# marcelm/cutadapt

Hardware: NVIDIA H100
Metric: reads/sec (150bp SE, 1 adapter, e=0.1) (higher is better)
Workload: dtype u8

## Files before the change

cutadapt_b200/csrc/cg_api.cu:

```cuda
#include <cuda_runtime.h>
#include <stdio.h>
#include <stdlib.h>
#include <string.h>

#include <algorithm>
#include <chrono>
#include <map>
#include <memory>
#include <string>
#include <type_traits>
#include <vector>

#include "../../include/cutadapt_b200.h"
#include "cg_hostpack.h"
#include <array>

#include "cg_gzip_core.cuh"
#include "cg_kernels.cuh"
#include "cg_jit.h"
#include "cg_setbuild.h"

static_assert(sizeof(cg_match) == 32 && sizeof(cg_match_rec) == 32, "cg_match must be 32 bytes");
static_assert(sizeof(CgAdapter) == 80 && sizeof(CgEntry) == 32 && sizeof(CgGroup) == 32 &&
                  sizeof(CgSetHeader) == 80, "table layout");

static thread_local std::string g_err;

static int fail(int code, const std::string &msg)
{
    g_err = msg;
    return code;
}
static int cuda_fail(cudaError_t e, const char *what)
{
    char buf[256];
    snprintf(buf, sizeof buf, "CUDA error in %s: %s", what, cudaGetErrorString(e));
    g_err = buf;
    return e == cudaErrorMemoryAllocation ? CG_ENOMEM : CG_ECUDA;
}
#define CU(x)                                                  \
    do {                                                       \
        cudaError_t _e = (x);                                  \
        if (_e != cudaSuccess) return cuda_fail(_e, #x);       \
    } while (0)

extern "C" int cg_version(void) { return CG_ABI_VERSION; }
extern "C" const char *cg_last_error(void) { return g_err.c_str(); }

template <class T, bool Pinned> class GrowBuf {
  public:
    T *p = nullptr;
    size_t cap = 0;
    GrowBuf() = default;
    GrowBuf(const GrowBuf &) = delete;
    GrowBuf &operator=(const GrowBuf &) = delete;
    GrowBuf(GrowBuf &&o) noexcept : p(o.p), cap(o.cap) { o.p = nullptr; o.cap = 0; }
    GrowBuf &operator=(GrowBuf &&o) noexcept
    {
        if (this != &o) {
            release();
            p = o.p; cap = o.cap;
            o.p = nullptr; o.cap = 0;
        }
        return *this;
    }
    ~GrowBuf() { release(); }
    int ensure(size_t n)
    {
        if (n <= cap) return CG_OK;
        release();
        size_t want = n + n / 4 + 64;
        cudaError_t e = Pinned ? cudaMallocHost((void **)&p, want * sizeof(T)) : cudaMalloc((void **)&p, want * sizeof(T));
        if (e != cudaSuccess) return cuda_fail(e, Pinned ? "cudaMallocHost" : "cudaMalloc");
        cap = want;
        return CG_OK;
    }

  private:
    void release()
    {
        if (p) Pinned ? cudaFreeHost(p) : cudaFree(p);
        p = nullptr; cap = 0;
    }
};
template <class T> using DevBuf = GrowBuf<T, false>;
template <class T> using PinBuf = GrowBuf<T, true>;
static_assert(!std::is_copy_constructible<DevBuf<uint8_t>>::value && !std::is_copy_constructible<PinBuf<uint8_t>>::value,
              "buffers own their memory: move them");

#define CG_N_LANES 3
struct Lane {
    cudaStream_t stream = nullptr;
    DevBuf<uint8_t> d_seq, d_qual, d_pack;
    DevBuf<uint64_t> d_exc;
    PinBuf<uint8_t> h_pack;
    PinBuf<uint64_t> h_exc;
    DevBuf<int64_t> d_offs;
    DevBuf<cg_match_rec> d_out;
    DevBuf<int32_t> d_qtrim;
    PinBuf<uint8_t> h_seq, h_qual;
    PinBuf<int64_t> h_offs;
    PinBuf<cg_match_rec> h_out;
    PinBuf<int32_t> h_qtrim;
    bool busy = false;
    cg_match_rec *dst_out = nullptr; size_t n_out = 0; bool out_bounced = false;
    int32_t *dst_qtrim = nullptr; size_t n_qtrim = 0; bool qtrim_bounced = false;
};

#define CG_ROWS_KINDS 3
struct FqRows {
    bool requested = false;
    bool gzip = false;
    int32_t n_entries = 0;
    std::vector<char> text;
    std::vector<int32_t> text_off;
    int64_t limit = -1;
    DevBuf<uint8_t> d_text, d_out, d_gz;
    DevBuf<int32_t> d_textoff, d_row;
    DevBuf<int64_t> d_rowoff;
    int64_t bytes = 0, bytes_plain = 0;
};

#define CG_FQ_SLOTS 4
struct FastqSlot {
    cudaStream_t stream = nullptr;
    bool busy = false;
    int64_t n_bytes = 0;
    DevBuf<uint8_t> d_in, d_out, d_seq, d_qual;
    DevBuf<uint32_t> d_tiles, d_nl;
    DevBuf<CgFastqRecord> d_rec;
    DevBuf<int32_t> d_len, d_interval, d_keep, d_outlen, d_qtrim, d_mask, d_adest, d_dmbytes, d_dest, d_pairkey, d_origin;
    DevBuf<uint8_t> d_destkeep;
    FqRows rows[CG_ROWS_KINDS];
    bool rows_ready = false;
    DevBuf<int64_t> d_dmbase;
    DevBuf<int64_t> d_offs, d_outoff;
    DevBuf<unsigned long long> d_scan;
    DevBuf<cg_match_rec> d_matches, d_matches_rc;
    DevBuf<uint8_t> d_isrc;
    DevBuf<uint8_t> d_norm;
    DevBuf<int32_t> d_faline;
    DevBuf<int64_t> d_faoff;
    DevBuf<unsigned long long> d_fqstats;
    DevBuf<int32_t> d_polya;
    PinBuf<unsigned long long> h_fqstats;
    DevBuf<int32_t> d_fold;
    DevBuf<unsigned long long> d_ilverr;
    DevBuf<CgGzPiece> d_gzpieces;
    DevBuf<uint8_t> d_gzslots, d_gzout;
    DevBuf<int32_t> d_gzsizes;
    DevBuf<int64_t> d_gzoff;
    int ilv = 0, ilv_peer = -1, ilv_format = 0;
    DevBuf<unsigned long long> d_counters;
    DevBuf<int> d_err;
    PinBuf<uint8_t> h_in, h_out;
    PinBuf<unsigned long long> h_counters;
};

struct GzinStream {
    DevBuf<uint8_t> d_gz, d_plain;
    PinBuf<uint8_t> h_gz;
    DevBuf<int32_t> d_counts, d_cand, d_members, d_flag;
    DevBuf<int64_t> d_offs;
    DevBuf<GuMember> d_res;
    DevBuf<long long> d_moff;
    DevBuf<unsigned long long> d_scan, d_small;
    DevBuf<uint32_t> d_tiles, d_nl;
    cudaEvent_t done = nullptr;
    long long carry = 0, consumed = 0, members = 0;
    long long pend_plain = 0, pend_consumed = 0, pend_members = 0;
    bool split = false;
    long long stride = CG_GZIN_STRIDE;
    struct Member { int in = 0, bitoff = 0, trailer = 0; uint32_t crc = 0; long long len = 0, start = 0; } mem, pmem;
    long long pend_respec = 0;
    DevBuf<uint8_t> d_win, d_pwin, d_wins;
    DevBuf<GuChunk> d_ch;
    DevBuf<long long> d_coff, d_room;
    DevBuf<uint16_t> d_sym;
    DevBuf<int32_t> d_redo;
    DevBuf<uint32_t> d_part;
    ~GzinStream() { if (done) cudaEventDestroy(done); }
};

struct FqStatsAcc {
    int32_t n_adapters = 0, max_len = 0, kmax = 0;
    std::vector<int64_t> v;
};

struct cg_ctx {
    int device = 0;
    cudaStream_t stream = nullptr;
    bool own_stream = false;
    int sm_count = 148;
    size_t smem_optin = 0;
    Lane lanes[CG_N_LANES];
    int *d_err = nullptr;
    uint8_t *d_enc = nullptr;
    double *d_phred = nullptr;
    DevBuf<uint32_t> scratch_p;
    DevBuf<int> scratch_w;
    DevBuf<unsigned long long> d_stats;
    DevBuf<uint4> tasks;
    DevBuf<uint4> tasks2, tasks3;
    DevBuf<uint2> stat_ents;
    unsigned long long *d_task_count = nullptr;
    DevBuf<cg_match_rec> pass_tmp;
    DevBuf<int32_t> view_base, view_back;
    long long launches = 0;
    std::vector<std::pair<cudaEvent_t, cudaEvent_t>> timing;
    std::vector<cudaEvent_t> event_pool;
    double timed_ms = 0.0;
    long long timed_n = 0;
    std::vector<std::array<cudaEvent_t, 4>> stage_events;
    double stage_ms[3] = {0, 0, 0};
    CgHostPool *pool = nullptr;
    std::vector<std::vector<uint64_t>> exc_scratch;
    long long h2d_bytes = 0, d2h_bytes = 0;
    double prof[8] = {0, 0, 0, 0, 0, 0, 0, 0};
    double pack_fraction = 0.6;
    double pack_ref_fraction = 0.6, pack_ref_rate = 0.0;
    int pack_dir = +1;
    bool pack_have_ref = false;
    int numa_node = -1;
    cudaEvent_t scratch_ev = nullptr;
    cudaStream_t scratch_stream = nullptr;
    bool scratch_busy = false;
    FastqSlot fq[CG_FQ_SLOTS];
    int fq_next = 0;
    std::map<int32_t, FqStatsAcc> fq_stats;
    int32_t fq_stats_next = 1;
    std::map<int32_t, GzinStream> gzin;
    int32_t gzin_next = 1;
};

struct cg_adapterset {
    cg_ctx *ctx = nullptr;
    CgBuiltSet host;
    uint8_t *d_blob = nullptr;
    uint64_t *d_masks = nullptr;
    CgEntry *d_entries = nullptr;
    uint8_t *d_index = nullptr;
    struct Pass {
        cg_adapterset *sub = nullptr;
        int group = 0, role = 0;
        int front_pass = -1;
        int map_off = 0;
    };
    std::vector<Pass> passes;
    std::vector<int32_t> pass_map;
    int32_t *d_pass_map = nullptr;
    CgSelectTables select_tables;
    mutable CgJitKernel *jit[2][2][2] = {};
    mutable int jit_state[2][2][2] = {};
    mutable long long plane_reads = 0;
    mutable std::string jit_error;
};

extern "C" int cg_ctx_create(int device, void *stream, cg_ctx **out)
{
    if (!out) return fail(CG_EINVAL, "cg_ctx_create: out is NULL");
    int count = 0;
    cudaError_t e = cudaGetDeviceCount(&count);
    if (e != cudaSuccess || count == 0)
        return fail(CG_ECUDA, std::string("no usable CUDA device (") + cudaGetErrorString(e) +
                                  "); cutadapt_b200 has no CPU fallback");
    if (device < 0 || device >= count) return fail(CG_EINVAL, "cg_ctx_create: device ordinal out of range");
    CU(cudaSetDevice(device));
    std::unique_ptr<cg_ctx, decltype(&cg_ctx_destroy)> c(new cg_ctx(), cg_ctx_destroy);
    c->device = device;
    cudaDeviceProp prop;
    CU(cudaGetDeviceProperties(&prop, device));
    c->sm_count = prop.multiProcessorCount;
    c->smem_optin = prop.sharedMemPerBlockOptin;
    if (stream) { c->stream = (cudaStream_t)stream; c->own_stream = false; }
    else { CU(cudaStreamCreateWithFlags(&c->stream, cudaStreamNonBlocking)); c->own_stream = true; }
    for (int i = 0; i < CG_N_LANES; ++i) CU(cudaStreamCreateWithFlags(&c->lanes[i].stream, cudaStreamNonBlocking));
    CU(cudaEventCreateWithFlags(&c->scratch_ev, cudaEventDisableTiming));
    CU(cudaMalloc((void **)&c->d_err, 16 * sizeof(int)));
    CU(cudaMemset(c->d_err, 0, 16 * sizeof(int)));
    CU(cudaMalloc((void **)&c->d_task_count, 64));
    CU(cudaMemset(c->d_task_count, 0, 64));
    CU(cudaMalloc((void **)&c->d_enc, 768));
    uint8_t enc[768];
    cg_build_enc_tables(enc);
    CU(cudaMemcpy(c->d_enc, enc, 768, cudaMemcpyHostToDevice));
    {
        double phred[256];
        cg_build_phred_table(phred);
        CU(cudaMalloc((void **)&c->d_phred, sizeof phred));
        CU(cudaMemcpy(c->d_phred, phred, sizeof phred, cudaMemcpyHostToDevice));
    }
    *out = c.release();
    return CG_OK;
}

static void resolve_timing(cg_ctx *c)
{
    for (auto &pr : c->timing) {
        float ms = 0.f;
        if (cudaEventSynchronize(pr.second) == cudaSuccess && cudaEventElapsedTime(&ms, pr.first, pr.second) == cudaSuccess) {
            c->timed_ms += ms; c->timed_n += 1;
        }
        c->event_pool.push_back(pr.first);
        c->event_pool.push_back(pr.second);
    }
    c->timing.clear();
}

extern "C" int cg_ctx_destroy(cg_ctx *c)
{
    if (!c) return CG_OK;
    cudaSetDevice(c->device);
    cudaDeviceSynchronize();
    resolve_timing(c);
    for (auto ev : c->event_pool) cudaEventDestroy(ev);
    delete c->pool;
    c->pool = nullptr;
    for (Lane &l : c->lanes)
        if (l.stream) cudaStreamDestroy(l.stream);
    for (FastqSlot &f : c->fq)
        if (f.stream) cudaStreamDestroy(f.stream);
    if (c->scratch_ev) cudaEventDestroy(c->scratch_ev);
    if (c->d_task_count) cudaFree(c->d_task_count);
    if (c->d_err) cudaFree(c->d_err);
    if (c->d_enc) cudaFree(c->d_enc);
    if (c->d_phred) cudaFree(c->d_phred);
    if (c->own_stream && c->stream) cudaStreamDestroy(c->stream);
    delete c;
    return CG_OK;
}

extern "C" int cg_ctx_synchronize(cg_ctx *c)
{
    if (!c) return fail(CG_EINVAL, "ctx is NULL");
    CU(cudaSetDevice(c->device));
    CU(cudaStreamSynchronize(c->stream));
    for (int i = 0; i < CG_N_LANES; ++i) CU(cudaStreamSynchronize(c->lanes[i].stream));
    return CG_OK;
}

extern "C" int64_t cg_ctx_launch_count(cg_ctx *c) { return c ? c->launches : 0; }

extern "C" int cg_ctx_stage_times(cg_ctx *c, double *out3, int reset)
{
    if (!c || !out3) return fail(CG_EINVAL, "cg_ctx_stage_times: NULL argument");
    CU(cudaSetDevice(c->device));
    for (auto &e : c->stage_events) {
        CU(cudaEventSynchronize(e[3]));
        for (int i = 0; i < 3; ++i) {
            float ms = 0;
            CU(cudaEventElapsedTime(&ms, e[i], e[i + 1]));
            c->stage_ms[i] += ms;
        }
        for (auto ev : e) cudaEventDestroy(ev);
    }
    c->stage_events.clear();
    for (int i = 0; i < 3; ++i) out3[i] = c->stage_ms[i];
    if (reset) c->stage_ms[0] = c->stage_ms[1] = c->stage_ms[2] = 0;
    return CG_OK;
}

extern "C" int cg_ctx_kernel_time(cg_ctx *c, double *total_ms, int64_t *launches, int reset)
{
    if (!c) return fail(CG_EINVAL, "ctx is NULL");
    CU(cudaSetDevice(c->device));
    resolve_timing(c);
    if (total_ms) *total_ms = c->timed_ms;
    if (launches) *launches = c->timed_n;
    if (reset) { c->timed_ms = 0.0; c->timed_n = 0; }
    return CG_OK;
}

static void destroy_passes(cg_adapterset *s)
{
    for (auto &p : s->passes) cg_adapterset_destroy(p.sub);
    s->passes.clear();
    s->pass_map.clear();
    if (s->d_pass_map) { cudaFree(s->d_pass_map); s->d_pass_map = nullptr; }
}

static int upload_set(cg_ctx *c, cg_adapterset *s)
{
    s->ctx = c;
    cudaError_t e = cudaSetDevice(c->device);
    if (e == cudaSuccess) e = cudaMalloc((void **)&s->d_blob, s->host.blob.size());
    if (e == cudaSuccess) e = cudaMemcpy(s->d_blob, s->host.blob.data(), s->host.blob.size(), cudaMemcpyHostToDevice);
    if (e == cudaSuccess) e = cudaMalloc((void **)&s->d_masks, s->host.masks64.size() * 8);
    if (e == cudaSuccess) e = cudaMemcpy(s->d_masks, s->host.masks64.data(), s->host.masks64.size() * 8, cudaMemcpyHostToDevice);
    if (e == cudaSuccess && !s->host.index_blob.empty()) {
        e = cudaMalloc((void **)&s->d_index, s->host.index_blob.size());
        if (e == cudaSuccess) e = cudaMemcpy(s->d_index, s->host.index_blob.data(), s->host.index_blob.size(), cudaMemcpyHostToDevice);
    }
    if (e != cudaSuccess) {
        if (s->d_blob) cudaFree(s->d_blob);
        if (s->d_masks) cudaFree(s->d_masks);
        if (s->d_index) cudaFree(s->d_index);
        s->d_blob = nullptr; s->d_masks = nullptr; s->d_index = nullptr;
        return cuda_fail(e, "adapter set upload");
    }
    return CG_OK;
}

extern "C" int cg_adapterset_create_indexed(cg_ctx *c, const cg_adapter_desc *adapters, int32_t n_adapters,
                                            const cg_group_desc *groups, int32_t n_groups,
                                            const cg_index_desc *indexes, int32_t n_indexes, cg_adapterset **out)
{
    if (!c || !out) return fail(CG_EINVAL, "cg_adapterset_create: NULL argument");
    cg_adapterset *s = new cg_adapterset();
    std::string err;
    int rc = cg_build_set(adapters, n_adapters, groups, n_groups, s->host, err, indexes, n_indexes);
    if (rc != CG_OK) { delete s; return fail(rc, err); }
    rc = upload_set(c, s);
    if (rc != CG_OK) { delete s; return rc; }
    CgMultiPlan plan;
    if (cg_plan_passes(adapters, n_adapters, groups, n_groups, indexes, n_indexes, plan, err) == CG_OK &&
        !plan.passes.empty()) {
        bool ok = true;
        for (auto &pp : plan.passes) {
            cg_adapterset::Pass P;
            P.group = pp.group; P.role = pp.role; P.front_pass = pp.front_pass; P.map_off = pp.map_off;
            P.sub = new cg_adapterset();
            P.sub->host = std::move(pp.set);
            if (upload_set(c, P.sub) != CG_OK) { delete P.sub; ok = false; break; }
            s->passes.push_back(P);
        }
        if (ok) {
            const CgSetHeader *H = (const CgSetHeader *)s->host.blob.data();
            cg_fill_select_tables((const CgGroup *)(s->host.blob.data() + H->groups_off), s->host.n_groups,
                                  s->host.slots, plan.passes, s->select_tables);
            s->pass_map = plan.pass_map;
            cudaError_t e = cudaMalloc((void **)&s->d_pass_map, s->pass_map.size() * sizeof(int32_t));
            if (e == cudaSuccess)
                e = cudaMemcpy(s->d_pass_map, s->pass_map.data(), s->pass_map.size() * sizeof(int32_t), cudaMemcpyHostToDevice);
            if (e != cudaSuccess) { cudaGetLastError(); ok = false; }
        }
        if (!ok) destroy_passes(s);
    }
    *out = s;
    return CG_OK;
}

extern "C" int cg_adapterset_create(cg_ctx *c, const cg_adapter_desc *adapters, int32_t n_adapters,
                                    const cg_group_desc *groups, int32_t n_groups, cg_adapterset **out)
{
    return cg_adapterset_create_indexed(c, adapters, n_adapters, groups, n_groups, nullptr, 0, out);
}

extern "C" int cg_adapterset_destroy(cg_adapterset *s)
{
    if (!s) return CG_OK;
    if (s->ctx) cudaSetDevice(s->ctx->device);
    if (s->d_blob) cudaFree(s->d_blob);
    if (s->d_masks) cudaFree(s->d_masks);
    if (s->d_index) cudaFree(s->d_index);
    for (int w = 0; w < 2; ++w)
        for (int q = 0; q < 2; ++q)
            for (int v = 0; v < 2; ++v) cg_jit_destroy(s->jit[w][q][v]);
    destroy_passes(s);
    delete s;
    return CG_OK;
}

extern "C" int cg_adapterset_jit_status(const cg_adapterset *s)
{
    if (!s) return 0;
    const cg_adapterset *t = (!s->passes.empty() && s->passes[0].sub) ? s->passes[0].sub : s;
    int st = 0;
    for (int w = 0; w < 2; ++w)
        for (int q = 0; q < 2; ++q)
            for (int v = 0; v < 2; ++v) {
                if (t->jit_state[w][q][v] == 1) st = 1;
                else if (t->jit_state[w][q][v] == -1 && st == 0) st = -1;
            }
    if (st == -1) g_err = "first-stage specialisation failed: " + t->jit_error;
    return st;
}

extern "C" int64_t cg_adapterset_jit_source(const cg_adapterset *s, int32_t plane_words, int32_t has_qual, int32_t stats,
                                            char *buf, int64_t cap)
{
    if (!s) return 0;
    const std::string src = cg_jit_pscan_source(s->host, plane_words, has_qual != 0, stats != 0);
    if (buf && cap > 0) {
        const size_t n = std::min<size_t>(src.size(), (size_t)cap - 1);
        memcpy(buf, src.data(), n);
        buf[n] = 0;
    }
    return (int64_t)src.size();
}

extern "C" int cg_adapterset_slots(const cg_adapterset *s) { return s ? s->host.slots : 0; }

extern "C" int cg_adapterset_effective_length(const cg_adapterset *s, int32_t adapter, int32_t *out)
{
    if (!s || !out || adapter < 0 || adapter >= s->host.n_adapters) return fail(CG_EINVAL, "bad adapter index");
    *out = s->host.effective_length[adapter];
    return CG_OK;
}

struct TrimSwitches {
    static bool is(const char *name, const char *value) { const char *e = getenv(name); return e && strcmp(e, value) == 0; }
    static long long at_least_1024(const char *e) { const long long v = e ? atoll(e) : 0; return v >= 1024 ? v : 0; }
    bool force_general = is("CUTADAPT_B200_KERNEL", "general");
    bool force_block = is("CUTADAPT_B200_KERNEL", "block");
    bool force_warp = is("CUTADAPT_B200_KERNEL", "warp");
    bool shiftand = is("CUTADAPT_B200_SCAN", "shiftand");
    bool no_band = getenv("CUTADAPT_B200_NO_BAND") != nullptr;
    bool no_light = getenv("CUTADAPT_B200_NO_LIGHT") != nullptr;
    bool no_index_kernel = getenv("CUTADAPT_B200_NO_INDEX_KERNEL") != nullptr;
    bool two_lists = getenv("CUTADAPT_B200_TWO_LISTS") != nullptr;
    bool task_bytes = getenv("CUTADAPT_B200_TASK_BYTES") != nullptr;
    bool no_band_lists = getenv("CUTADAPT_B200_NO_BAND_LISTS") != nullptr;
    bool stage_times = getenv("CUTADAPT_B200_STAGE_TIMES") != nullptr;
    bool jit_never = is("CUTADAPT_B200_JIT", "0"), jit_always = is("CUTADAPT_B200_JIT", "1");
    long long sub_reads = at_least_1024(getenv("CUTADAPT_B200_SUB_READS"));
};

struct StatsRequest { unsigned long long *d_stats; int max_len, kmax; };

enum class TrimKind { Index, Light, Split, Warp, Fast, Generic, MultiPass };

struct TrimSchedule {
    TrimKind kind = TrimKind::Generic;
    int tile_cap = 0, mini_cap = 0, carry_slot = 0;
    size_t smem = 0;
    int occ = 0;
    bool simple = false;
    size_t list_smem = 0;
    int plan_occ = 0, run_occ = 0;
    int plane_w = 0, plane_rec = 0;
    long long sub = 0;
    CgJitKernel *jit = nullptr;
    int jit_occ = 0;
    bool fuse_stats = false;
};

static int choose_schedule(cg_ctx *c, const cg_adapterset *s, int64_t n_reads, int max_read_len, const cg_params *p,
                           bool has_view, const StatsRequest *stats, const TrimSwitches &sw, TrimSchedule &d)
{
    const CgBuiltSet &h = s->host;
    const int times = p->times < 1 ? 1 : p->times;
    const bool want_q = p->quality_trim != 0 || p->nextseq_trim != 0;
    if (!s->passes.empty() && times == 1 && !sw.force_general) {
        d.kind = TrimKind::MultiPass;
        d.sub = sw.sub_reads ? sw.sub_reads : 32LL << 20;
        return CG_OK;
    }
    if (h.all_indexed && !want_q && !h.any_wide && h.max_m + 1 <= CG_LIGHT_ROWS && !sw.force_general && !sw.no_light) {
        d.kind = times == 1 && !has_view && h.slots == 1 && !sw.no_index_kernel ? TrimKind::Index : TrimKind::Light;
        d.sub = 64LL << 20;
        return CG_OK;
    }
    const uint32_t blob_bytes = (uint32_t)h.blob.size();
    const long long tile_cap = ((long long)CG_NT * max_read_len + 32 + 15) / 16 * 16;
    bool fast = !h.any_wide && max_read_len <= CG_PACKED_MAX_N && tile_cap < (1 << 24);
    if (fast) {
        d.tile_cap = (int)tile_cap;
        d.smem = cg_fast_smem_bytes(blob_bytes, d.tile_cap, h.max_m + 1, want_q);
        fast = d.smem <= c->smem_optin;
    }
    d.simple = fast && h.simple_ok && times == 1 && !sw.force_general;
    if (fast) {
        CU(cg_fast_occupancy(want_q, d.simple, d.smem, &d.occ));
        fast = d.occ >= 1;
    }
    d.kind = fast ? TrimKind::Fast : TrimKind::Generic;
    const long long mini = ((long long)32 * max_read_len + 32 + 15) / 16 * 16;
    if (d.simple && h.max_m <= 32 && sw.force_warp && mini < (1 << 20)) {
        d.mini_cap = (int)mini;
        d.carry_slot = (int)(((long long)max_read_len + 4 + 15) / 16 * 16 + 16);
        const size_t wsmem = cg_warp_smem_bytes(blob_bytes, d.mini_cap, d.carry_slot, want_q);
        int wocc = 0;
        if (wsmem <= c->smem_optin) CU(cg_warp_occupancy(want_q, wsmem, &wocc));
        if (wocc >= 1) { d.kind = TrimKind::Warp; d.smem = wsmem; d.occ = wocc; }
        return CG_OK;
    }
    if (!d.simple || h.max_m > 64 || sw.force_block || sw.force_warp || mini >= (1 << 20)) return CG_OK;
    const CgSetHeader *hdr = (const CgSetHeader *)h.blob.data();
    if (hdr->plane_count > 0 && max_read_len <= 256 && !sw.shiftand) d.plane_w = max_read_len <= 160 ? 5 : 8;
    const long long cslot = ((long long)max_read_len + 4 + 15) / 16 * 16 + 32;
    d.mini_cap = (int)mini;
    d.carry_slot = (int)(d.plane_w ? std::max<long long>(cslot, 16LL * (2 * d.plane_w + 1) + 16) : cslot);
    size_t scan_smem = d.plane_w ? cg_pscan_smem_bytes(blob_bytes, d.mini_cap, want_q)
                                 : cg_scan_smem_bytes(blob_bytes, d.mini_cap, want_q);
    d.list_smem = cg_dp_smem_bytes(blob_bytes, d.carry_slot);
    if (scan_smem > c->smem_optin || d.list_smem > c->smem_optin) return CG_OK;
    int scan_occ = 0;
    if (d.plane_w) CU(cg_pscan_occupancy(want_q, d.plane_w, false, scan_smem, &scan_occ));
    else CU(cg_scan_occupancy(want_q, scan_smem, &scan_occ));
    CU(cg_list_occupancy(true, h.max_m, false, d.list_smem, &d.plan_occ));
    CU(cg_list_occupancy(false, h.max_m, false, d.list_smem, &d.run_occ));
    if (scan_occ < 1 || d.plan_occ < 1 || d.run_occ < 1) return CG_OK;
    if (d.plane_w && stats && !has_view && h.n_adapters == 1 && times == 1 && h.slots == 1 && !want_q && !sw.two_lists &&
        stats->max_len <= 4096 && cg_stats_entries_smem_bytes(stats->max_len, stats->kmax) <= 48 * 1024) {
        const size_t fsmem = cg_pscan_smem_bytes(blob_bytes, d.mini_cap, want_q, stats->max_len);
        int focc = 0;
        if (fsmem <= c->smem_optin) CU(cg_pscan_occupancy(want_q, d.plane_w, true, fsmem, &focc));
        int pocc = 0, rocc = 0;
        CU(cg_list_occupancy(true, h.max_m, true, d.list_smem, &pocc));
        CU(cg_list_occupancy(false, h.max_m, true, d.list_smem, &rocc));
        d.fuse_stats = focc >= 1 && focc >= scan_occ && pocc >= d.plan_occ && rocc >= d.run_occ;
        if (d.fuse_stats) { scan_smem = fsmem; scan_occ = focc; }
    }
    if (d.plane_w) {
        const int wi = d.plane_w <= 5 ? 0 : 1, qi = want_q ? 1 : 0, vi = d.fuse_stats ? 1 : 0;
        s->plane_reads += n_reads;
        if (!sw.jit_never && s->jit_state[wi][qi][vi] == 0 && (sw.jit_always || s->plane_reads >= (4LL << 20))) {
            std::string err;
            s->jit[wi][qi][vi] = cg_jit_build_pscan(h, d.plane_w, want_q, d.fuse_stats, err);
            s->jit_state[wi][qi][vi] = s->jit[wi][qi][vi] ? 1 : -1;
            if (!s->jit[wi][qi][vi]) s->jit_error = err;
        }
        if (!sw.jit_never && s->jit_state[wi][qi][vi] == 1) {
            d.jit_occ = cg_jit_occupancy(s->jit[wi][qi][vi], CG_NT, scan_smem);
            if (d.jit_occ >= 1) d.jit = s->jit[wi][qi][vi];
        }
    }
    d.kind = TrimKind::Split;
    d.smem = scan_smem; d.occ = scan_occ;
    d.sub = sw.sub_reads ? sw.sub_reads : (d.plane_w && sw.task_bytes) ? (16LL << 20) : (32LL << 20);
    d.sub = std::min<long long>(d.sub, 1LL << 31);
    d.plane_rec = d.plane_w ? (sw.task_bytes ? 4 + 2 * d.plane_w + 1 : 4) : 2;
    return CG_OK;
}

static int trim_grid(const cg_ctx *c, int blocks_per_sm, long long need)
{
    return (int)std::max<long long>(1, std::min<long long>((long long)blocks_per_sm * c->sm_count, need));
}

static int launch_index(cg_ctx *c, const CgKernelArgs &a, const TrimSchedule &d, cudaStream_t st)
{
    int rc = c->tasks.ensure((size_t)((std::min<long long>(a.n_reads, d.sub) + 3) / 4));
    if (rc != CG_OK) return rc;
    for (long long r0 = 0; r0 < a.n_reads; r0 += d.sub) {
        const long long n_sub = std::min<long long>(d.sub, a.n_reads - r0);
        CgKernelArgs b = a;
        b.offsets = a.offsets + r0; b.n_reads = n_sub; b.out = a.out + (size_t)r0 * a.slots;
        b.tasks = c->tasks.p; b.task_count = c->d_task_count;
        CU(cudaMemsetAsync(c->d_task_count, 0, sizeof(unsigned long long), st));
        CU(cg_launch_index(b, trim_grid(c, 16, (n_sub + CG_NT - 1) / CG_NT), st));
        c->launches += 2;
    }
    return CG_OK;
}

static int launch_split(cg_ctx *c, const cg_adapterset *s, const CgKernelArgs &a, const TrimSchedule &d,
                        const TrimSwitches &sw, cudaStream_t st)
{
    const long long cap = std::min<long long>(a.n_reads, d.sub);
    int rc = c->tasks.ensure((size_t)cap * d.plane_rec);
    if (rc == CG_OK) rc = c->tasks2.ensure((size_t)cap * 4);
    if (rc == CG_OK) rc = c->tasks3.ensure((size_t)cap * 4);
    if (rc == CG_OK && d.fuse_stats) rc = c->stat_ents.ensure((size_t)cap);
    if (rc != CG_OK) return rc;
    unsigned long long *cnt = c->d_task_count;
    for (long long r0 = 0; r0 < a.n_reads; r0 += d.sub) {
        const long long n_sub = std::min<long long>(d.sub, a.n_reads - r0);
        CgKernelArgs b = a;
        b.offsets = a.offsets + r0;
        b.n_reads = n_sub;
        b.out = a.out + (size_t)r0 * a.times * a.slots;
        b.qtrim = a.qtrim ? a.qtrim + 2 * r0 : nullptr;
        b.view = a.view ? a.view + 2 * r0 : nullptr;
        b.task_cap = n_sub;
        CU(cudaMemsetAsync(cnt, 0, 8 * sizeof(unsigned long long), st));
        const long long need = ((n_sub + 31) / 32 + 3) / 4;
        std::array<cudaEvent_t, 4> sev = {nullptr, nullptr, nullptr, nullptr};
        if (sw.stage_times && c->stage_events.size() < 4096) {
            for (auto &e : sev) CU(cudaEventCreate(&e));
            CU(cudaEventRecord(sev[0], st));
        }
        b.tasks = c->tasks.p; b.task_count = cnt;
        b.task_rec = d.plane_rec;
        b.task_count_b = (d.plane_w && sw.two_lists) ? cnt + 4 : nullptr;
        if (d.plane_w && d.jit) {
            const int rcj = cg_jit_launch(d.jit, trim_grid(c, d.jit_occ, need), CG_NT, d.smem, (void *)st, &b);
            if (rcj != 0) return fail(CG_ECUDA, "launch of the specialised first stage failed (CUresult " + std::to_string(rcj) + ")");
        }
        else if (d.plane_w) CU(cg_launch_pscan(b, a.quality_trim != 0, d.plane_w, trim_grid(c, d.occ, need), d.smem, st));
        else CU(cg_launch_scan(b, a.quality_trim != 0, trim_grid(c, d.occ, need), d.smem, st));
        if (sev[0]) CU(cudaEventRecord(sev[1], st));
        b.stat_ents = c->stat_ents.p; b.stat_count = cnt + 6;
        b.tasks2 = c->tasks2.p; b.task2_count = cnt + 1;
        b.tasks3 = c->tasks3.p; b.task3_count = cnt + 2;
        b.task2_count_b = (CG_RUN_BAND && d.plane_w && !sw.no_band_lists) ? cnt + 5 : nullptr;
        CU(cg_launch_list(b, true, s->host.max_m, trim_grid(c, d.plan_occ, need), d.list_smem, st));
        c->launches += 2;
        if (d.plane_w) {
            CgKernelArgs b2 = b;
            b2.tasks = c->tasks3.p; b2.task_count = cnt + 2; b2.task_rec = 2;
            b2.tasks3 = nullptr; b2.task3_count = cnt + 3; b2.task_count_b = nullptr;
            CU(cg_launch_list(b2, true, s->host.max_m, trim_grid(c, d.plan_occ, need), d.list_smem, st));
            CU(cudaMemsetAsync(cnt + 2, 0, sizeof(unsigned long long), st));
            c->launches += 1;
        }
        if (sev[0]) CU(cudaEventRecord(sev[2], st));
        uint4 *lists[2] = {c->tasks2.p, c->tasks3.p};
        for (int round = 0; round < 4; ++round) {
            const int in = round & 1, outl = in ^ 1;
            if (round > 0) CU(cudaMemsetAsync(cnt + 1 + outl, 0, sizeof(unsigned long long), st));
            b.tasks = lists[in]; b.task_count = cnt + 1 + in;
            b.task_count_b = round == 0 ? b.task2_count_b : nullptr;
            b.tasks2 = lists[outl]; b.task2_count = cnt + 1 + outl;
            if (round == 0) b.task2_count_b = nullptr;
            else b.task_count_b = nullptr;
            CU(cg_launch_list(b, false, s->host.max_m, trim_grid(c, d.run_occ, need), d.list_smem, st));
            c->launches += 1;
        }
        if (sev[0]) { CU(cudaEventRecord(sev[3], st)); c->stage_events.push_back(sev); }
        if (d.fuse_stats) {
            CU(cg_launch_stats_entries(c->stat_ents.p, cnt + 6, n_sub, a.stats_max_len, a.stats_kmax, a.stats, st));
            c->launches += 1;
        }
    }
    return CG_OK;
}

static int launch_generic(cg_ctx *c, CgKernelArgs a, cudaStream_t st)
{
    const int block = 128;
    long long threads = (long long)c->sm_count * 8 * block;
    const long long per_thread = (long long)a.col_rows * 16;
    while (threads > 32 * block && threads * per_thread > (1LL << 30)) threads /= 2;
    if (threads > ((a.n_reads + block - 1) / block) * block) threads = ((a.n_reads + block - 1) / block) * block;
    int rc = c->scratch_p.ensure((size_t)threads * a.col_rows);
    if (rc != CG_OK) return rc;
    rc = c->scratch_w.ensure((size_t)threads * a.col_rows * 3);
    if (rc != CG_OK) return rc;
    a.scratch_p = c->scratch_p.p; a.scratch_w = c->scratch_w.p; a.scratch_stride = threads;
    CU(cg_launch_generic(a, (int)(threads / block), block, st));
    c->launches += 1;
    return CG_OK;
}

static int trim_pass(cg_ctx *c, const cg_adapterset *s, const uint8_t *d_seq, const uint8_t *d_qual,
                     const int64_t *d_offsets, int64_t n_reads, int max_read_len, const cg_params *p,
                     cg_match_rec *d_out, int32_t *d_qtrim, const int32_t *d_view, cudaStream_t st, bool timed,
                     const StatsRequest *stats, const TrimSwitches &sw, bool *stats_counted);

static int launch_multi_pass(cg_ctx *c, const cg_adapterset *s, const CgKernelArgs &a, int max_read_len,
                             const cg_params *p, const TrimSchedule &d, const TrimSwitches &sw, cudaStream_t st)
{
    const bool want_q = a.quality_trim != 0;
    const int np = (int)s->passes.size();
    const long long cap = std::min<long long>(a.n_reads, d.sub);
    int rc = c->pass_tmp.ensure((size_t)cap * np);
    if (rc != CG_OK) return rc;
    bool any_linked = false;
    for (auto &P : s->passes) any_linked = any_linked || P.role == 1;
    if (any_linked) { rc = c->view_back.ensure((size_t)cap * 2); if (rc != CG_OK) return rc; }
    if (want_q && !a.qtrim) { rc = c->view_base.ensure((size_t)cap * 2); if (rc != CG_OK) return rc; }

    CgSelectArgs sel;
    memset(&sel, 0, sizeof sel);
    sel.tmp = c->pass_tmp.p; sel.stride = cap; sel.pass_map = s->d_pass_map;
    sel.t = s->select_tables;

    for (long long r0 = 0; r0 < a.n_reads; r0 += d.sub) {
        const long long n_sub = std::min<long long>(d.sub, a.n_reads - r0);
        const int64_t *offs = a.offsets + r0;
        int32_t *qt = want_q ? (a.qtrim ? a.qtrim + 2 * r0 : c->view_base.p) : nullptr;
        const int32_t *base_view = nullptr;
        for (int pi = 0; pi < np; ++pi) {
            const auto &P = s->passes[pi];
            cg_match_rec *tmp = c->pass_tmp.p + (size_t)pi * cap;
            cg_params pp = *p;
            pp.times = 1;
            const int32_t *view = base_view;
            if (P.role == 1) {
                CU(cg_launch_linked_view(c->pass_tmp.p + (size_t)P.front_pass * cap, base_view, offs, n_sub,
                                         c->view_back.p, st));
                c->launches += 1;
                view = c->view_back.p;
            }
            const bool trims = want_q && pi == 0;
            if (!trims) { pp.quality_trim = 0; pp.nextseq_trim = 0; }
            rc = trim_pass(c, P.sub, a.seq, trims ? a.qual : nullptr, offs, n_sub, max_read_len, &pp, tmp,
                           trims ? qt : nullptr, trims ? nullptr : view, st, false, nullptr, sw, nullptr);
            if (rc != CG_OK) return rc;
            if (trims) base_view = qt;
        }
        sel.n_reads = n_sub;
        sel.out = a.out + (size_t)r0 * s->host.slots;
        CU(cg_launch_select(sel, st));
        c->launches += 1;
    }
    return CG_OK;
}

static int trim_pass(cg_ctx *c, const cg_adapterset *s, const uint8_t *d_seq, const uint8_t *d_qual,
                     const int64_t *d_offsets, int64_t n_reads, int max_read_len, const cg_params *p,
                     cg_match_rec *d_out, int32_t *d_qtrim, const int32_t *d_view, cudaStream_t st, bool timed,
                     const StatsRequest *stats, const TrimSwitches &sw, bool *stats_counted)
{
    const bool want_q = p->quality_trim != 0 || p->nextseq_trim != 0;
    if (want_q && !d_qual) return fail(CG_ENOQUAL, "Cannot do quality trimming when no qualities are available");
    TrimSchedule d;
    int rc = choose_schedule(c, s, n_reads, max_read_len, p, d_view != nullptr, stats, sw, d);
    if (rc != CG_OK) return rc;
    CgKernelArgs a;
    memset(&a, 0, sizeof a);
    a.blob = s->d_blob; a.blob_bytes = (uint32_t)s->host.blob.size();
    a.masks64 = s->d_masks; a.enc = c->d_enc; a.index = s->d_index;
    a.seq = d_seq; a.qual = want_q ? d_qual : nullptr; a.offsets = d_offsets; a.n_reads = n_reads;
    a.quality_trim = (p->quality_trim ? 1 : 0) | (p->nextseq_trim ? 2 : 0);
    a.cutoff_front = p->cutoff_front; a.cutoff_back = p->cutoff_back;
    a.qbase = (p->quality_base & 255) | (int)((unsigned)p->nextseq_cutoff << 8);
    a.times = p->times < 1 ? 1 : p->times; a.slots = s->host.slots;
    a.out = d_out; a.qtrim = d_qtrim; a.view = d_view; a.err_flag = c->d_err;
    a.col_rows = s->host.max_m + 1; a.no_band = sw.no_band;
    a.tile_cap = d.tile_cap; a.mini_cap = d.mini_cap; a.carry_slot = d.carry_slot;
    if (d.fuse_stats) { a.stats = stats->d_stats; a.stats_max_len = stats->max_len; a.stats_kmax = stats->kmax; }
    cudaEvent_t ev[2] = {nullptr, nullptr};
    if (timed && c->timing.size() < 8192) {
        for (cudaEvent_t &e : ev) {
            if (!c->event_pool.empty()) { e = c->event_pool.back(); c->event_pool.pop_back(); }
            else CU(cudaEventCreate(&e));
        }
        CU(cudaEventRecord(ev[0], st));
    }
    switch (d.kind) {
    case TrimKind::Index: rc = launch_index(c, a, d, st); break;
    case TrimKind::Light:
        CU(cg_launch_light(a, trim_grid(c, 16, (n_reads + CG_NT - 1) / CG_NT), st));
        c->launches += 1;
        break;
    case TrimKind::Split: rc = launch_split(c, s, a, d, sw, st); break;
    case TrimKind::Warp:
        CU(cg_launch_warp(a, want_q, trim_grid(c, d.occ, ((n_reads + 31) / 32 + 3) / 4), d.smem, st));
        c->launches += 1;
        break;
    case TrimKind::Fast:
        CU(cg_launch_fast(a, want_q, d.simple, trim_grid(c, d.occ, (n_reads + CG_NT - 1) / CG_NT), d.smem, st));
        c->launches += 1;
        break;
    case TrimKind::Generic: rc = launch_generic(c, a, st); break;
    case TrimKind::MultiPass: rc = launch_multi_pass(c, s, a, max_read_len, p, d, sw, st); break;
    }
    if (rc != CG_OK) return rc;
    if (ev[0]) {
        CU(cudaEventRecord(ev[1], st));
        c->timing.emplace_back(ev[0], ev[1]);
    }
    if (stats_counted) *stats_counted = d.fuse_stats;
    return CG_OK;
}

extern "C" int cg_locate_debug(cg_ctx *c, const cg_adapter_desc *adapter, const uint8_t *query, int32_t n,
                               int32_t *cost, int32_t *score, int32_t *result8)
{
    if (!c || !adapter || !cost || !score || !result8 || n < 0 || (n && !query))
        return fail(CG_EINVAL, "cg_locate_debug: bad argument");
    if (adapter->kind != CG_KIND_ALIGNER) return fail(CG_EINVAL, "cg_locate_debug: only aligner adapters have a DP matrix");
    for (int32_t i = 0; i < n; ++i) if (query[i] & 0x80) return fail(CG_ENONASCII, "String must contain only ASCII characters");
    CU(cudaSetDevice(c->device));
    cg_adapter_desc d = *adapter;
    d.n_kmer_entries = 0; d.kmer_entries = nullptr; d.kmer_masks = nullptr; d.reverse_read = 0;
    cg_group_desc g;
    memset(&g, 0, sizeof g);
    g.type = CG_GROUP_SINGLE; g.a0 = 0; g.a1 = -1;
    CgBuiltSet set;
    std::string err;
    int rc = cg_build_set(&d, 1, &g, 1, set, err);
    if (rc != CG_OK) return fail(rc, err);
    const int m = set.max_m;
    const size_t cells = (size_t)(m + 1) * ((size_t)n + 1);
    DevBuf<uint8_t> d_blob, d_query;
    DevBuf<int> d_scratch;
    DevBuf<int32_t> d_mat, d_res;
    if ((rc = d_blob.ensure(set.blob.size())) != CG_OK || (rc = d_query.ensure((size_t)n + 16)) != CG_OK ||
        (rc = d_scratch.ensure(3 * ((size_t)m + 2))) != CG_OK || (rc = d_mat.ensure(2 * cells)) != CG_OK ||
        (rc = d_res.ensure(8)) != CG_OK)
        return rc;
    std::vector<int32_t> none(2 * cells, CG_DEBUG_NONE);
    CU(cudaMemcpy(d_blob.p, set.blob.data(), set.blob.size(), cudaMemcpyHostToDevice));
    if (n) CU(cudaMemcpy(d_query.p, query, (size_t)n, cudaMemcpyHostToDevice));
    CU(cudaMemcpy(d_mat.p, none.data(), 2 * cells * sizeof(int32_t), cudaMemcpyHostToDevice));
    CU(cg_launch_locate_debug(d_blob.p, c->d_enc, d_query.p, n, d_scratch.p, d_mat.p, d_mat.p + cells, d_res.p, c->stream));
    c->launches += 1;
    CU(cudaStreamSynchronize(c->stream));
    CU(cudaMemcpy(cost, d_mat.p, cells * sizeof(int32_t), cudaMemcpyDeviceToHost));
    CU(cudaMemcpy(score, d_mat.p + cells, cells * sizeof(int32_t), cudaMemcpyDeviceToHost));
    CU(cudaMemcpy(result8, d_res.p, 8 * sizeof(int32_t), cudaMemcpyDeviceToHost));
    return CG_OK;
}

static int launch_trim(cg_ctx *c, const cg_adapterset *s, const uint8_t *d_seq, const uint8_t *d_qual,
                       const int64_t *d_offsets, int64_t n_reads, int max_read_len, const cg_params *p,
                       cg_match_rec *d_out, int32_t *d_qtrim, cudaStream_t st, bool timed,
                       const StatsRequest *stats = nullptr, bool *stats_counted = nullptr)
{
    if (n_reads <= 0) return CG_OK;
    if (c->scratch_busy && c->scratch_stream != st) CU(cudaStreamWaitEvent(st, c->scratch_ev, 0));
    const int rc = trim_pass(c, s, d_seq, d_qual, d_offsets, n_reads, max_read_len, p, d_out, d_qtrim, nullptr, st, timed,
                             stats, TrimSwitches(), stats_counted);
    CU(cudaEventRecord(c->scratch_ev, st));
    c->scratch_busy = true;
    c->scratch_stream = st;
    return rc;
}

static int launch_trim_with_stats(cg_ctx *c, const cg_adapterset *s, const uint8_t *d_seq, const uint8_t *d_qual,
                                  const int64_t *d_offsets, int64_t n_reads, int max_read_len, const cg_params *p,
                                  cg_match_rec *d_out, int32_t *d_qtrim, cudaStream_t st, bool timed,
                                  unsigned long long *d_stats, int stats_max_len, int stats_kmax)
{
    if (n_reads <= 0) return CG_OK;
    const StatsRequest req = {d_stats, stats_max_len, stats_kmax};
    bool counted = false;
    const int rc = launch_trim(c, s, d_seq, d_qual, d_offsets, n_reads, max_read_len, p, d_out, d_qtrim, st, timed, &req,
                               &counted);
    if (rc != CG_OK || counted) return rc;
    const int times = p->times < 1 ? 1 : p->times;
    CU(cg_launch_stats(d_seq, d_offsets, n_reads, (p->quality_trim || p->nextseq_trim) && d_qtrim, times, s->host.slots,
                       d_out, d_qtrim, s->host.n_adapters, stats_max_len, stats_kmax, d_stats, st));
    c->launches += 1;
    return CG_OK;
}

static int check_err_flag(cg_ctx *c)
{
    int flags[2] = {0, 0};
    CU(cudaMemcpy(flags, c->d_err, sizeof flags, cudaMemcpyDeviceToHost));
    if (flags[0]) {
        cudaMemset(c->d_err, 0, sizeof(int));
        return fail(CG_ENONASCII, "String must contain only ASCII characters");
    }
    return CG_OK;
}

extern "C" int cg_process_batch_device(cg_ctx *c, const cg_adapterset *s, const uint8_t *d_seq,
                                       const uint8_t *d_qual, const int64_t *d_offsets, int64_t n_reads,
                                       int32_t max_read_len, const cg_params *p, cg_match *d_matches,
                                       int32_t *d_qtrim)
{
    if (!c || !s || !p || !d_seq || !d_offsets || !d_matches) return fail(CG_EINVAL, "cg_process_batch_device: NULL argument");
    if (s->ctx != c) return fail(CG_EINVAL, "adapter set belongs to another context");
    if (((uintptr_t)d_seq & 15) || (d_qual && ((uintptr_t)d_qual & 15)))
        return fail(CG_EINVAL, "device sequence/quality buffers must be 16-byte aligned");
    if (n_reads < 0) return fail(CG_EINVAL, "n_reads < 0");
    CU(cudaSetDevice(c->device));
    if (max_read_len <= 0) {
        CU(cudaMemsetAsync(c->d_err + 1, 0, sizeof(int), c->stream));
        CU(cg_launch_max_len(d_offsets, n_reads, c->d_err + 1, c->stream));
        c->launches += 1;
        CU(cudaMemcpyAsync(&max_read_len, c->d_err + 1, sizeof(int), cudaMemcpyDeviceToHost, c->stream));
        CU(cudaStreamSynchronize(c->stream));
    }
    return launch_trim(c, s, d_seq, d_qual, d_offsets, n_reads, max_read_len, p, (cg_match_rec *)d_matches,
                       d_qtrim, c->stream, true);
}

extern "C" int cg_process_batch_device_stats(cg_ctx *c, const cg_adapterset *s, const uint8_t *d_seq,
                                             const uint8_t *d_qual, const int64_t *d_offsets, int64_t n_reads,
                                             int32_t max_read_len, const cg_params *p, cg_match *d_matches,
                                             int32_t *d_qtrim, int32_t stats_max_len, int32_t stats_kmax, int64_t *d_stats)
{
    if (!c || !s || !p || !d_seq || !d_offsets || !d_matches || !d_stats || stats_max_len < 0 || stats_kmax < 0)
        return fail(CG_EINVAL, "cg_process_batch_device_stats: bad argument");
    if (s->ctx != c) return fail(CG_EINVAL, "adapter set belongs to another context");
    if (((uintptr_t)d_seq & 15) || (d_qual && ((uintptr_t)d_qual & 15)))
        return fail(CG_EINVAL, "device sequence/quality buffers must be 16-byte aligned");
    if (n_reads < 0) return fail(CG_EINVAL, "n_reads < 0");
    if ((p->quality_trim || p->nextseq_trim) && !d_qtrim)
        return fail(CG_EINVAL, "cg_process_batch_device_stats: quality trimming needs d_qtrim (the statistics read it)");
    CU(cudaSetDevice(c->device));
    if (max_read_len <= 0) {
        CU(cudaMemsetAsync(c->d_err + 1, 0, sizeof(int), c->stream));
        CU(cg_launch_max_len(d_offsets, n_reads, c->d_err + 1, c->stream));
        c->launches += 1;
        CU(cudaMemcpyAsync(&max_read_len, c->d_err + 1, sizeof(int), cudaMemcpyDeviceToHost, c->stream));
        CU(cudaStreamSynchronize(c->stream));
    }
    return launch_trim_with_stats(c, s, d_seq, d_qual, d_offsets, n_reads, max_read_len, p, (cg_match_rec *)d_matches,
                                  d_qtrim, c->stream, true, (unsigned long long *)d_stats, stats_max_len, stats_kmax);
}

static void parallel_copy(cg_ctx *c, void *dst, const void *src, size_t n);

static bool is_pinned(const void *p)
{
    if (!p) return false;
    cudaPointerAttributes at;
    if (cudaPointerGetAttributes(&at, p) != cudaSuccess) { cudaGetLastError(); return false; }
    return at.type == cudaMemoryTypeHost;
}

static int lane_finish(cg_ctx *c, Lane &l)
{
    if (!l.busy) return CG_OK;
    CU(cudaStreamSynchronize(l.stream));
    if (l.out_bounced && l.n_out) memcpy(l.dst_out, l.h_out.p, l.n_out * sizeof(cg_match_rec));
    if (l.qtrim_bounced && l.n_qtrim) memcpy(l.dst_qtrim, l.h_qtrim.p, l.n_qtrim * sizeof(int32_t));
    l.busy = false;
    return CG_OK;
}

struct OffsetScan { int64_t max_len = 0; bool uniform = true, valid = true; };
static OffsetScan scan_offsets_part(const int64_t *offsets, int64_t len0, int64_t a, int64_t b)
{
    OffsetScan o;
    for (int64_t r = a; r < b; ++r) {
        const int64_t len = offsets[r + 1] - offsets[r];
        if (len < 0 || len > 2000000000LL) o.valid = false;
        if (len > o.max_len) o.max_len = len;
        o.uniform = o.uniform && len == len0;
    }
    return o;
}
static void scan_merge(OffsetScan &t, const OffsetScan &o)
{
    t.max_len = std::max(t.max_len, o.max_len);
    t.uniform = t.uniform && o.uniform;
    t.valid = t.valid && o.valid;
}
static const int64_t SCAN_JOB = 1 << 15;
static OffsetScan scan_offsets(cg_ctx *c, const int64_t *offsets, int64_t r0, int64_t r1)
// ... 2607 lines not shown
```

Baseline: 7.552 billion.

## Overlap scan of next sub-batch with list stages on a second stream

Splits the split-trim schedule into sub-batches with triple-buffered task lists and counters, running the scan kernel on the main stream and the planning/run list kernels on a separate stream, synchronised by events. Each side gets a reduced grid occupancy so both can co-run on the SMs. Sub-batch size drops to 16M reads when overlap is possible. This trades extra buffer memory, event overhead and smaller per-kernel grids for concurrency between the scan and list stages.

```diff
diff --git a/cutadapt_b200/csrc/cg_api.cu b/cutadapt_b200/csrc/cg_api.cu
--- a/cutadapt_b200/csrc/cg_api.cu
+++ b/cutadapt_b200/csrc/cg_api.cu
@@ -87,6 +87,14 @@
 template <class T> using PinBuf = GrowBuf<T, true>;
 static_assert(!std::is_copy_constructible<DevBuf<uint8_t>>::value && !std::is_copy_constructible<PinBuf<uint8_t>>::value,
               "buffers own their memory: move them");
+
+#ifndef CG_SPLIT_SUB_READS
+#define CG_SPLIT_SUB_READS (16LL << 20)
+#endif
+#define CG_LIST_SETS 3
+#ifndef CG_OVERLAP_SCAN_EIGHTHS
+#define CG_OVERLAP_SCAN_EIGHTHS 4
+#endif
 
 #define CG_N_LANES 3
 struct Lane {
@@ -200,10 +208,15 @@
     DevBuf<uint32_t> scratch_p;
     DevBuf<int> scratch_w;
     DevBuf<unsigned long long> d_stats;
-    DevBuf<uint4> tasks;
-    DevBuf<uint4> tasks2, tasks3;
-    DevBuf<uint2> stat_ents;
+    struct ListSet {
+        DevBuf<uint4> tasks;
+        DevBuf<uint4> tasks2, tasks3;
+        DevBuf<uint2> stat_ents;
+        cudaEvent_t done = nullptr;
+    } lists[CG_LIST_SETS];
     unsigned long long *d_task_count = nullptr;
+    cudaStream_t list_stream = nullptr;
+    cudaEvent_t scan_done = nullptr;
     DevBuf<cg_match_rec> pass_tmp;
     DevBuf<int32_t> view_base, view_back;
     long long launches = 0;
@@ -211,7 +224,7 @@
     std::vector<cudaEvent_t> event_pool;
     double timed_ms = 0.0;
     long long timed_n = 0;
-    std::vector<std::array<cudaEvent_t, 4>> stage_events;
+    std::vector<std::array<cudaEvent_t, 5>> stage_events;
     double stage_ms[3] = {0, 0, 0};
     CgHostPool *pool = nullptr;
     std::vector<std::vector<uint64_t>> exc_scratch;
@@ -276,10 +289,13 @@
     else { CU(cudaStreamCreateWithFlags(&c->stream, cudaStreamNonBlocking)); c->own_stream = true; }
     for (int i = 0; i < CG_N_LANES; ++i) CU(cudaStreamCreateWithFlags(&c->lanes[i].stream, cudaStreamNonBlocking));
     CU(cudaEventCreateWithFlags(&c->scratch_ev, cudaEventDisableTiming));
+    CU(cudaStreamCreateWithFlags(&c->list_stream, cudaStreamNonBlocking));
+    CU(cudaEventCreateWithFlags(&c->scan_done, cudaEventDisableTiming));
+    for (auto &L : c->lists) CU(cudaEventCreateWithFlags(&L.done, cudaEventDisableTiming));
     CU(cudaMalloc((void **)&c->d_err, 16 * sizeof(int)));
     CU(cudaMemset(c->d_err, 0, 16 * sizeof(int)));
-    CU(cudaMalloc((void **)&c->d_task_count, 64));
-    CU(cudaMemset(c->d_task_count, 0, 64));
+    CU(cudaMalloc((void **)&c->d_task_count, 64 * CG_LIST_SETS));
+    CU(cudaMemset(c->d_task_count, 0, 64 * CG_LIST_SETS));
     CU(cudaMalloc((void **)&c->d_enc, 768));
     uint8_t enc[768];
     cg_build_enc_tables(enc);
@@ -321,6 +337,10 @@
     for (FastqSlot &f : c->fq)
         if (f.stream) cudaStreamDestroy(f.stream);
     if (c->scratch_ev) cudaEventDestroy(c->scratch_ev);
+    if (c->scan_done) cudaEventDestroy(c->scan_done);
+    for (auto &L : c->lists)
+        if (L.done) cudaEventDestroy(L.done);
+    if (c->list_stream) cudaStreamDestroy(c->list_stream);
     if (c->d_task_count) cudaFree(c->d_task_count);
     if (c->d_err) cudaFree(c->d_err);
     if (c->d_enc) cudaFree(c->d_enc);
@@ -346,10 +366,12 @@
     if (!c || !out3) return fail(CG_EINVAL, "cg_ctx_stage_times: NULL argument");
     CU(cudaSetDevice(c->device));
     for (auto &e : c->stage_events) {
-        CU(cudaEventSynchronize(e[3]));
+        CU(cudaEventSynchronize(e[1]));
+        CU(cudaEventSynchronize(e[4]));
+        const int from[3] = {0, 2, 3};
         for (int i = 0; i < 3; ++i) {
             float ms = 0;
-            CU(cudaEventElapsedTime(&ms, e[i], e[i + 1]));
+            CU(cudaEventElapsedTime(&ms, e[from[i]], e[from[i] + 1]));
             c->stage_ms[i] += ms;
         }
         for (auto ev : e) cudaEventDestroy(ev);
@@ -528,6 +550,8 @@
     bool simple = false;
     size_t list_smem = 0;
     int plan_occ = 0, run_occ = 0;
+    bool overlap = false;
+    int ov_occ[3] = {0, 0, 0};
     int plane_w = 0, plane_rec = 0;
     long long sub = 0;
     CgJitKernel *jit = nullptr;
@@ -618,8 +642,18 @@
     }
     d.kind = TrimKind::Split;
     d.smem = scan_smem; d.occ = scan_occ;
-    d.sub = sw.sub_reads ? sw.sub_reads : (d.plane_w && sw.task_bytes) ? (16LL << 20) : (32LL << 20);
+    const int k = CG_OVERLAP_SCAN_EIGHTHS;
+    const int ov_plan = d.plan_occ * (8 - k) / 8, ov_run = d.run_occ * (8 - k) / 8;
+    const bool can_overlap = d.plane_w && ov_plan >= 2 && ov_run >= 2;
+    d.sub = sw.sub_reads ? sw.sub_reads : (can_overlap || (d.plane_w && sw.task_bytes)) ? CG_SPLIT_SUB_READS
+                                                                                         : (32LL << 20);
     d.sub = std::min<long long>(d.sub, 1LL << 31);
+    d.overlap = can_overlap && n_reads > d.sub;
+    if (d.overlap) {
+        d.ov_occ[0] = std::max(1, (d.jit ? d.jit_occ : d.occ) * k / 8);
+        d.ov_occ[1] = ov_plan;
+        d.ov_occ[2] = ov_run;
+    }
     d.plane_rec = d.plane_w ? (sw.task_bytes ? 4 + 2 * d.plane_w + 1 : 4) : 2;
     return CG_OK;
 }
@@ -631,13 +665,13 @@
 
 static int launch_index(cg_ctx *c, const CgKernelArgs &a, const TrimSchedule &d, cudaStream_t st)
 {
-    int rc = c->tasks.ensure((size_t)((std::min<long long>(a.n_reads, d.sub) + 3) / 4));
+    int rc = c->lists[0].tasks.ensure((size_t)((std::min<long long>(a.n_reads, d.sub) + 3) / 4));
     if (rc != CG_OK) return rc;
     for (long long r0 = 0; r0 < a.n_reads; r0 += d.sub) {
         const long long n_sub = std::min<long long>(d.sub, a.n_reads - r0);
         CgKernelArgs b = a;
         b.offsets = a.offsets + r0; b.n_reads = n_sub; b.out = a.out + (size_t)r0 * a.slots;
-        b.tasks = c->tasks.p; b.task_count = c->d_task_count;
+        b.tasks = c->lists[0].tasks.p; b.task_count = c->d_task_count;
         CU(cudaMemsetAsync(c->d_task_count, 0, sizeof(unsigned long long), st));
         CU(cg_launch_index(b, trim_grid(c, 16, (n_sub + CG_NT - 1) / CG_NT), st));
         c->launches += 2;
@@ -649,14 +683,24 @@
                         const TrimSwitches &sw, cudaStream_t st)
 {
     const long long cap = std::min<long long>(a.n_reads, d.sub);
-    int rc = c->tasks.ensure((size_t)cap * d.plane_rec);
-    if (rc == CG_OK) rc = c->tasks2.ensure((size_t)cap * 4);
-    if (rc == CG_OK) rc = c->tasks3.ensure((size_t)cap * 4);
-    if (rc == CG_OK && d.fuse_stats) rc = c->stat_ents.ensure((size_t)cap);
-    if (rc != CG_OK) return rc;
-    unsigned long long *cnt = c->d_task_count;
-    for (long long r0 = 0; r0 < a.n_reads; r0 += d.sub) {
-        const long long n_sub = std::min<long long>(d.sub, a.n_reads - r0);
+    const long long n_subs = (a.n_reads + d.sub - 1) / d.sub;
+    const int sets = d.overlap ? CG_LIST_SETS : 1;
+    for (long long k = 0; k < std::min<long long>(n_subs, sets); ++k) {
+        cg_ctx::ListSet &L = c->lists[k];
+        int rc = L.tasks.ensure((size_t)cap * d.plane_rec);
+        if (rc == CG_OK) rc = L.tasks2.ensure((size_t)cap * 4);
+        if (rc == CG_OK) rc = L.tasks3.ensure((size_t)cap * 4);
+        if (rc == CG_OK && d.fuse_stats) rc = L.stat_ents.ensure((size_t)cap);
+        if (rc != CG_OK) return rc;
+    }
+    const cudaStream_t ls = d.overlap ? c->list_stream : st;
+    for (long long j = 0; j < n_subs; ++j) {
+        const long long r0 = j * d.sub, n_sub = std::min<long long>(d.sub, a.n_reads - r0);
+        cg_ctx::ListSet &L = c->lists[j % sets];
+        unsigned long long *cnt = c->d_task_count + 8 * (j % sets);
+        const int scan_occ = d.overlap && j > 0 ? d.ov_occ[0] : d.jit ? d.jit_occ : d.occ;
+        const bool lists_shared = d.overlap && j + 1 < n_subs;
+        const int plan_occ = lists_shared ? d.ov_occ[1] : d.plan_occ, run_occ = lists_shared ? d.ov_occ[2] : d.run_occ;
         CgKernelArgs b = a;
         b.offsets = a.offsets + r0;
         b.n_reads = n_sub;
@@ -664,56 +708,64 @@
         b.qtrim = a.qtrim ? a.qtrim + 2 * r0 : nullptr;
         b.view = a.view ? a.view + 2 * r0 : nullptr;
         b.task_cap = n_sub;
+        if (ls != st && j >= sets) CU(cudaStreamWaitEvent(st, L.done, 0));
         CU(cudaMemsetAsync(cnt, 0, 8 * sizeof(unsigned long long), st));
         const long long need = ((n_sub + 31) / 32 + 3) / 4;
-        std::array<cudaEvent_t, 4> sev = {nullptr, nullptr, nullptr, nullptr};
+        std::array<cudaEvent_t, 5> sev = {nullptr, nullptr, nullptr, nullptr, nullptr};
         if (sw.stage_times && c->stage_events.size() < 4096) {
             for (auto &e : sev) CU(cudaEventCreate(&e));
             CU(cudaEventRecord(sev[0], st));
         }
-        b.tasks = c->tasks.p; b.task_count = cnt;
+        b.tasks = L.tasks.p; b.task_count = cnt;
         b.task_rec = d.plane_rec;
         b.task_count_b = (d.plane_w && sw.two_lists) ? cnt + 4 : nullptr;
         if (d.plane_w && d.jit) {
-            const int rcj = cg_jit_launch(d.jit, trim_grid(c, d.jit_occ, need), CG_NT, d.smem, (void *)st, &b);
+            const int rcj = cg_jit_launch(d.jit, trim_grid(c, scan_occ, need), CG_NT, d.smem, (void *)st, &b);
             if (rcj != 0) return fail(CG_ECUDA, "launch of the specialised first stage failed (CUresult " + std::to_string(rcj) + ")");
         }
-        else if (d.plane_w) CU(cg_launch_pscan(b, a.quality_trim != 0, d.plane_w, trim_grid(c, d.occ, need), d.smem, st));
-        else CU(cg_launch_scan(b, a.quality_trim != 0, trim_grid(c, d.occ, need), d.smem, st));
+        else if (d.plane_w) CU(cg_launch_pscan(b, a.quality_trim != 0, d.plane_w, trim_grid(c, scan_occ, need), d.smem, st));
+        else CU(cg_launch_scan(b, a.quality_trim != 0, trim_grid(c, scan_occ, need), d.smem, st));
         if (sev[0]) CU(cudaEventRecord(sev[1], st));
-        b.stat_ents = c->stat_ents.p; b.stat_count = cnt + 6;
-        b.tasks2 = c->tasks2.p; b.task2_count = cnt + 1;
-        b.tasks3 = c->tasks3.p; b.task3_count = cnt + 2;
+        if (ls != st) {
+            CU(cudaEventRecord(c->scan_done, st));
+            CU(cudaStreamWaitEvent(ls, c->scan_done, 0));
+        }
+        if (sev[0]) CU(cudaEventRecord(sev[2], ls));
+        b.stat_ents = L.stat_ents.p; b.stat_count = cnt + 6;
+        b.tasks2 = L.tasks2.p; b.task2_count = cnt + 1;
+        b.tasks3 = L.tasks3.p; b.task3_count = cnt + 2;
         b.task2_count_b = (CG_RUN_BAND && d.plane_w && !sw.no_band_lists) ? cnt + 5 : nullptr;
-        CU(cg_launch_list(b, true, s->host.max_m, trim_grid(c, d.plan_occ, need), d.list_smem, st));
+        CU(cg_launch_list(b, true, s->host.max_m, trim_grid(c, plan_occ, need), d.list_smem, ls));
         c->launches += 2;
         if (d.plane_w) {
             CgKernelArgs b2 = b;
-            b2.tasks = c->tasks3.p; b2.task_count = cnt + 2; b2.task_rec = 2;
+            b2.tasks = L.tasks3.p; b2.task_count = cnt + 2; b2.task_rec = 2;
             b2.tasks3 = nullptr; b2.task3_count = cnt + 3; b2.task_count_b = nullptr;
-            CU(cg_launch_list(b2, true, s->host.max_m, trim_grid(c, d.plan_occ, need), d.list_smem, st));
-            CU(cudaMemsetAsync(cnt + 2, 0, sizeof(unsigned long long), st));
+            CU(cg_launch_list(b2, true, s->host.max_m, trim_grid(c, plan_occ, need), d.list_smem, ls));
+            CU(cudaMemsetAsync(cnt + 2, 0, sizeof(unsigned long long), ls));
             c->launches += 1;
         }
-        if (sev[0]) CU(cudaEventRecord(sev[2], st));
-        uint4 *lists[2] = {c->tasks2.p, c->tasks3.p};
+        if (sev[0]) CU(cudaEventRecord(sev[3], ls));
+        uint4 *lists[2] = {L.tasks2.p, L.tasks3.p};
         for (int round = 0; round < 4; ++round) {
             const int in = round & 1, outl = in ^ 1;
-            if (round > 0) CU(cudaMemsetAsync(cnt + 1 + outl, 0, sizeof(unsigned long long), st));
+            if (round > 0) CU(cudaMemsetAsync(cnt + 1 + outl, 0, sizeof(unsigned long long), ls));
             b.tasks = lists[in]; b.task_count = cnt + 1 + in;
             b.task_count_b = round == 0 ? b.task2_count_b : nullptr;
             b.tasks2 = lists[outl]; b.task2_count = cnt + 1 + outl;
             if (round == 0) b.task2_count_b = nullptr;
             else b.task_count_b = nullptr;
-            CU(cg_launch_list(b, false, s->host.max_m, trim_grid(c, d.run_occ, need), d.list_smem, st));
+            CU(cg_launch_list(b, false, s->host.max_m, trim_grid(c, run_occ, need), d.list_smem, ls));
             c->launches += 1;
         }
-        if (sev[0]) { CU(cudaEventRecord(sev[3], st)); c->stage_events.push_back(sev); }
+        if (sev[0]) { CU(cudaEventRecord(sev[4], ls)); c->stage_events.push_back(sev); }
         if (d.fuse_stats) {
-            CU(cg_launch_stats_entries(c->stat_ents.p, cnt + 6, n_sub, a.stats_max_len, a.stats_kmax, a.stats, st));
+            CU(cg_launch_stats_entries(L.stat_ents.p, cnt + 6, n_sub, a.stats_max_len, a.stats_kmax, a.stats, ls));
             c->launches += 1;
         }
-    }
+        if (ls != st) CU(cudaEventRecord(L.done, ls));
+    }
+    if (ls != st) CU(cudaStreamWaitEvent(st, c->lists[(n_subs - 1) % sets].done, 0));
     return CG_OK;
 }
 
```

Result: faster. 7.762 billion, median of 6 (+2.8%).
